# lhoangan/arap_flow

Measured on AMD Instinct MI355X. Metric: ARAP solve+warp frames/sec at 854x480 mesh, higher is better.
Workload: dtype f32; 1 GPU; configs[1]: single 854x480 DAVIS-shaped frame, single-segment mask, fd=1; schedule 19/8/400; segments_per_frame=1, fd=1, parallelism=frames sharded, no collective, grid_vertices_per_frame=409920

## Files before the change

### arap_flow_amd/csrc/arap_resident.h

```cpp
#pragma once
#include <type_traits>
#include "arap_device.h"

namespace arap {

constexpr int RES_WGS = 512;
constexpr int RES_MAX_GROUPS = RES_WGS;
constexpr int RES_THREADS = 256;
constexpr int RES_SLOTS = 9;
constexpr int RES_TILES_PER_WG = RES_SLOTS;
constexpr int RT_X = 32, RT_Y = 8;
constexpr int RES_ZX = 2 * RT_X + 2 * RT_Y;
constexpr int RES_ZG = 2 * RES_ZX;
constexpr int RES_MAX_L = 32000;
static_assert(RT_X * RT_Y == RES_THREADS && RT_Y == 2 * (RES_THREADS / 64), "one vertex per lane, two rows per wavefront");
constexpr int RES_MAX_HALO = RES_TILES_PER_WG * (2 * RT_X + 2 * RT_Y);
constexpr int RES_HALO_PER_THREAD = (RES_MAX_HALO + RES_THREADS - 1) / RES_THREADS;
constexpr int RES_MAX_TILES = RES_WGS * RES_TILES_PER_WG;
constexpr int LROW = RT_X + 2;
constexpr int LROWS = RT_Y + 2;
constexpr int LPLANE = LROW * LROWS;
constexpr int LTILE = 5 * LPLANE;
constexpr int RES_LDS_BYTES = RES_TILES_PER_WG * LTILE * 4
                              + ((RES_MAX_HALO * 8 + 15) / 16) * 16
                              + RES_TILES_PER_WG * 8 + 8 + 384
                              + RES_TILES_PER_WG * RES_ZX * 16;
static_assert(2 * ((RES_LDS_BYTES + 1279) / 1280 * 1280) <= 160 * 1024, "two workgroups per CU");
#ifndef RES_HALO_REG_SLOTS
#define RES_HALO_REG_SLOTS 8
#endif
#ifndef RES_WREG_SLOTS
#define RES_WREG_SLOTS 7
#endif
#ifndef RES_WREG_8
#define RES_WREG_8 4
#endif
#ifndef RES_WREG_9
#define RES_WREG_9 4
#endif
#ifndef RES_WREG_FIT
#define RES_WREG_FIT 9
#endif
#ifndef RES_WREG_FIT_FLAT
#define RES_WREG_FIT_FLAT 9
#endif
#ifndef RES_WPIN
#define RES_WPIN 1
#endif
#ifndef RES_PREG_SLOTS
#define RES_PREG_SLOTS 7
#endif
#ifndef RES_PREG_SLOTS_FLAT
#define RES_PREG_SLOTS_FLAT 7
#endif
#ifndef RES_CSREG_SLOTS
#define RES_CSREG_SLOTS 7
#endif
#ifndef RES_CSREG_SLOTS_FLAT
#define RES_CSREG_SLOTS_FLAT 7
#endif
#ifndef RES_HPREG_SLOTS
#define RES_HPREG_SLOTS 6
#endif
#ifndef RES_HPREG_SLOTS_FLAT
#define RES_HPREG_SLOTS_FLAT 7
#endif
#ifndef RES_SWEEP1
#define RES_SWEEP1 1
#endif
#ifndef RES_WREG_8_FLAT
#define RES_WREG_8_FLAT 4
#endif
#ifndef RES_WREG_9_FLAT
#define RES_WREG_9_FLAT RES_WREG_9
#endif
#ifndef RES_PUB_MASK
#define RES_PUB_MASK 1
#endif
#ifndef RES_Z16
#define RES_Z16 1
#endif
#ifndef RES_FIRST_LOOK
#define RES_FIRST_LOOK 5
#endif
#ifndef RES_FIRST_LOOK_2
#define RES_FIRST_LOOK_2 14
#endif
#ifndef RES_FIRST_LOOK_X
#define RES_FIRST_LOOK_X 20
#endif
#ifndef RES_OWN_LOCAL
#define RES_OWN_LOCAL 1
#endif
#ifndef RES_POLL_SLEEP
#define RES_POLL_SLEEP 1
#endif
constexpr unsigned RES_SPIN_LIMIT = 1u << 18;
#ifndef RES_GRAN_STRIDE
#define RES_GRAN_STRIDE 2
#endif
constexpr int RES_GS = RES_GRAN_STRIDE;
constexpr int RES_GRAN_UNITS = 2 * RES_WGS;
constexpr int RES_GRAN_L1 = 2 * RES_GRAN_UNITS * RES_GS;
constexpr int RES_GRAN2_STRIDE = 16;
constexpr int RES_GRAN2_GROUP = 2 * 8 * RES_GRAN2_STRIDE;
constexpr int RES_GRAN_X = RES_GRAN_L1 + 4 * RES_GRAN2_GROUP;
constexpr int RES_GRAN_PER_LAUNCH = RES_GRAN_X + RES_GRAN_L1;
#ifndef RES_FLAT_MAX_RUNS
#define RES_FLAT_MAX_RUNS 2
#endif

constexpr int RES_SUMS_ANY = 0, RES_SUMS_FLAT = 1, RES_SUMS_COUNT = 2;

struct ResWg {
    int slot;
    int rank;
    int wgs;
    int gran;
};

struct ResDev {
    const int* tilelist;
    const int* ntiles;
    const int* tilepos;
    const int* bandx0;
    unsigned long long* zx;
    int rtX, rtY;
    unsigned long long* gran;
    unsigned* err;
    const ResWg* wgmap;
    int allow_fast;
    int force_fail;
    int flat_runs;
    int nowait;
    int fuse_update;
    unsigned long long* stamps;
};

typedef __attribute__((address_space(1))) unsigned long long gu64;
typedef __attribute__((address_space(1))) unsigned gu32;

__device__ __forceinline__ int border_entry(int x, int y)
{
    return y == 0 ? x : (y == RT_Y - 1 ? RT_X + x : (x == 0 ? 2 * RT_X + y : (x == RT_X - 1 ? 2 * RT_X + RT_Y + y : -1)));
}
__device__ __forceinline__ void st_tagged(unsigned long long* p, unsigned hi , float v, bool fast)
{
    const unsigned long long g = ((unsigned long long)hi << 32) | __float_as_uint(v);
    if (fast) __hip_atomic_store(p, g, __ATOMIC_RELAXED, __HIP_MEMORY_SCOPE_WORKGROUP);
    else __hip_atomic_store(p, g, __ATOMIC_RELAXED, __HIP_MEMORY_SCOPE_AGENT);
}
typedef unsigned v4u_t __attribute__((__vector_size__(4 * sizeof(unsigned))));
__device__ __forceinline__ void ld_zentry(const unsigned long long* zx_b, __amdgpu_buffer_rsrc_t zrs, unsigned gi,
                                          unsigned long long (&h)[2])
{
    if (RES_Z16) {
        const v4u_t w = __builtin_amdgcn_raw_buffer_load_b128(zrs, (int)(gi * 8u), 0, 16 );
        h[0] = ((unsigned long long)w[1] << 32) | w[0];
        h[1] = ((unsigned long long)w[3] << 32) | w[2];
    } else {
        const unsigned long long* q_ = (const unsigned long long*)((const char*)zx_b + (size_t)(gi * 8u));
#pragma unroll
        for (int c = 0; c < 2; ++c) h[c] = __hip_atomic_load(q_ + c, __ATOMIC_RELAXED, __HIP_MEMORY_SCOPE_AGENT);
    }
}
#define RES_GRANULE_FENCE() asm volatile("" ::: "memory")
typedef float v2f_t __attribute__((ext_vector_type(2)));
__device__ __forceinline__ float2 fma2(float2 a, float2 b, float2 c)
{
    const v2f_t r = __builtin_elementwise_fma((v2f_t){a.x, a.y}, (v2f_t){b.x, b.y}, (v2f_t){c.x, c.y});
    return make_float2(r.x, r.y);
}
template <int BITNO>
__device__ __forceinline__ float keep_if(unsigned f, float v)
{
    int m;
    asm("v_bfe_i32 %0, %1, %2, 1" : "=v"(m) : "v"(f), "n"(BITNO));
    return __uint_as_float(__float_as_uint(v) & (unsigned)m);
}

template <int BITNO>
__device__ __forceinline__ float keep_if_here(unsigned f, float v)
{
    int m;
    asm volatile("v_bfe_i32 %0, %1, %2, 1" : "=v"(m) : "v"(f), "n"(BITNO));
    return __uint_as_float(__float_as_uint(v) & (unsigned)m);
}

__device__ __forceinline__ void fma_into(float& p, float b, float z)
{
    asm("v_fma_f32 %0, %1, %0, %2" : "+v"(p) : "v"(b), "v"(z));
}

__device__ __forceinline__ double block_sum_uniform(double t)
{
    return __hiloint2double(__builtin_amdgcn_readlane(__double2hiint(t), 3), __builtin_amdgcn_readlane(__double2loint(t), 3));
}

__device__ __forceinline__ int res_publishes(bool fast, bool flavour)
{
    int s_ = (((threadIdx.x & 63) >> 1) == 1 && fast == flavour) ? 1 : 0;
    asm volatile("" : "+v"(s_));
    return s_;
}

template <bool ONE = false, bool PUBMASK = false>
__device__ __forceinline__ bool group_sum(double part, unsigned epoch, unsigned long long* gran_group, int rank,
                                          int wgs, float* bcast , unsigned* err, float& out,
                                          bool fast = false, double* out_d = nullptr, bool nowait = false,
                                          unsigned long long* tm = nullptr ,
                                          unsigned long long* tarr = nullptr ,
                                          int pubf = 0, int pubs = 0)
{
    const int wave = threadIdx.x >> 6, lane = threadIdx.x & 63;
    unsigned long long c0 = 0ull, c1;
    if (wave == 0) {
        if (tm) c0 = __builtin_amdgcn_s_memtime();
        if (tarr) *tarr += __builtin_amdgcn_s_memrealtime();
        __builtin_amdgcn_s_setprio(3);
        unsigned long long* buf = gran_group + (size_t)(epoch & 1u) * wgs * RES_GS;
        if (PUBMASK) {
            const unsigned long long bits = (unsigned long long)__double_as_longlong(part);
            const unsigned hw = lane == 2 ? (unsigned)bits : (unsigned)(bits >> 32);
            const unsigned long long gv = ((unsigned long long)epoch << 32) | hw;
            if (pubf) __hip_atomic_store(buf + rank * RES_GS + (lane - 2), gv, __ATOMIC_RELAXED, __HIP_MEMORY_SCOPE_WORKGROUP);
            if (pubs) __hip_atomic_store(buf + rank * RES_GS + (lane - 2), gv, __ATOMIC_RELAXED, __HIP_MEMORY_SCOPE_AGENT);
        } else if ((lane >> 1) == 1) {
            const unsigned long long bits = (unsigned long long)__double_as_longlong(part);
            const unsigned hw = lane == 2 ? (unsigned)bits : (unsigned)(bits >> 32);
            const unsigned long long gv = ((unsigned long long)epoch << 32) | hw;
            if (fast)
                __hip_atomic_store(buf + rank * RES_GS + (lane - 2), gv, __ATOMIC_RELAXED, __HIP_MEMORY_SCOPE_WORKGROUP);
            else
                __hip_atomic_store(buf + rank * RES_GS + (lane - 2), gv, __ATOMIC_RELAXED, __HIP_MEMORY_SCOPE_AGENT);
        }
        part = block_sum_uniform(part);
        double v = 0.0;
        bool ok = false;
        if (tm) { c1 = __builtin_amdgcn_s_memtime(); tm[0] += c1 - c0; c0 = c1; }
        __builtin_amdgcn_s_sleep(RES_FIRST_LOOK);
        const bool own1 = RES_OWN_LOCAL && lane == rank;
        const bool look = ONE && lane < wgs && !own1;
        const double idle = own1 ? part : 0.0;
        const __amdgpu_buffer_rsrc_t grs = __builtin_amdgcn_make_buffer_rsrc((void*)gran_group, 0, ONE ? 2 * wgs * RES_GS * 8 : 0, 0x00020000);
        const int qoff = (int)(((epoch & 1u) * (unsigned)wgs + (unsigned)lane) * (RES_GS * 8u));
        v4u_t w = {(unsigned)__double2loint(idle), epoch, (unsigned)__double2hiint(idle), epoch};
        const unsigned limit = nowait ? 1u : RES_SPIN_LIMIT;
        for (unsigned spins = 0; spins < limit; ++spins) {
            if (tm) tm[3] += 1;
            if (ONE) {
                RES_GRANULE_FENCE();
                if (look) w = __builtin_amdgcn_raw_buffer_load_b128(grs, qoff, 0, 16 );
                const bool late = w[1] != epoch || w[3] != epoch;
                v = __hiloint2double((int)w[2], (int)w[0]);
                ok = __builtin_amdgcn_ballot_w64(late) == 0ull;
                if (ok) break;
                if (RES_POLL_SLEEP) __builtin_amdgcn_s_sleep(1);
                continue;
            }
            v = 0.0;
            bool mine_ok = true;
            for (int m = lane; m < wgs; m += 64) {
                const unsigned long long lo = __hip_atomic_load(buf + RES_GS * m, __ATOMIC_RELAXED, __HIP_MEMORY_SCOPE_AGENT);
                const unsigned long long hi =
                    __hip_atomic_load(buf + RES_GS * m + 1, __ATOMIC_RELAXED, __HIP_MEMORY_SCOPE_AGENT);
                const bool own = RES_OWN_LOCAL && m == rank;
                mine_ok = mine_ok && (own || ((unsigned)(lo >> 32) == epoch && (unsigned)(hi >> 32) == epoch));
                v += own ? part : __longlong_as_double((long long)((hi << 32) | (lo & 0xffffffffull)));
            }
            ok = __builtin_amdgcn_ballot_w64(!mine_ok) == 0ull;
            if (ok) break;
            if (RES_POLL_SLEEP) __builtin_amdgcn_s_sleep(1);
        }
        ok = ok || nowait;
        if (tm) { c1 = __builtin_amdgcn_s_memtime(); tm[1] += c1 - c0; c0 = c1; asm volatile("" : "+v"(v)); }
        v = wave_sum_l63_full(v);
        if (tm) {
            asm volatile("" :: "v"(v));
            c1 = __builtin_amdgcn_s_memtime(); tm[4] += c1 - c0;
        }
        if (lane == 63) {
            *(float2*)(bcast + 2 * (epoch & 1u)) = make_float2((float)v, ok ? 1.0f : 0.0f);
            if (out_d) *out_d = v;
            if (!ok) atomicExch(err, 0xDEAD0000u | (epoch & 0xffffu));
        }
        __builtin_amdgcn_s_setprio(0);
        if (tm) { c1 = __builtin_amdgcn_s_memtime(); tm[2] += c1 - c0; c0 = c1; }
    }
    __syncthreads();
    const float2 bc = *(const float2*)(bcast + 2 * (epoch & 1u));
    out = bc.x;
    if (tm && wave == 0) {
        asm volatile("s_waitcnt lgkmcnt(0)" ::: "memory");
        tm[5] += __builtin_amdgcn_s_memtime() - c0;
    }
    return bc.y != 0.0f;
}

__device__ __forceinline__ bool group_sum_h(double part, unsigned epoch, unsigned long long* gran_group,
                                            unsigned long long* gran2 , int rank, int wgs,
                                            float* bcast, unsigned* err, float& out, bool subfast)
{
    const int wave = threadIdx.x >> 6, lane = threadIdx.x & 63;
    if (wave == 0) {
        __builtin_amdgcn_s_setprio(3);
        const int sub = rank >> 6, srank = rank & 63, nsub = wgs >> 6;
        unsigned long long* buf = gran_group + (size_t)sub * (128 * RES_GS) + (size_t)(epoch & 1u) * (64 * RES_GS);
        part = __hiloint2double(__builtin_amdgcn_readfirstlane(__double2hiint(part)),
                                __builtin_amdgcn_readfirstlane(__double2loint(part)));
        if (lane < 2) {
            const unsigned long long bits = (unsigned long long)__double_as_longlong(part);
            const unsigned hw = lane == 0 ? (unsigned)bits : (unsigned)(bits >> 32);
            const unsigned long long gv = ((unsigned long long)epoch << 32) | hw;
            if (subfast)
                __hip_atomic_store(buf + srank * RES_GS + lane, gv, __ATOMIC_RELAXED, __HIP_MEMORY_SCOPE_WORKGROUP);
            else
                __hip_atomic_store(buf + srank * RES_GS + lane, gv, __ATOMIC_RELAXED, __HIP_MEMORY_SCOPE_AGENT);
        }
        double v = 0.0;
        bool ok = false;
// ... 67 lines not shown
                if (subfast)
                    __hip_atomic_store(bufl + srank * RES_GS + lane, gv, __ATOMIC_RELAXED, __HIP_MEMORY_SCOPE_WORKGROUP);
                else
                    __hip_atomic_store(bufl + srank * RES_GS + lane, gv, __ATOMIC_RELAXED, __HIP_MEMORY_SCOPE_AGENT);
            } else {
                __hip_atomic_store(bufx + rank * RES_GS + (lane & 1), gv, __ATOMIC_RELAXED, __HIP_MEMORY_SCOPE_AGENT);
            }
        }
        double v = 0.0;
        bool ok = false;
        __builtin_amdgcn_s_sleep(RES_FIRST_LOOK_X);
        for (unsigned spins = 0; spins < RES_SPIN_LIMIT; ++spins) {
            v = 0.0;
            bool mine_ok = true;
            for (int r = 0; r < nsub; ++r) {
                if (r * 64 + lane >= wgs) break;
                const unsigned long long* src = r == sub ? bufl + RES_GS * lane : bufx + RES_GS * (r * 64 + lane);
                const unsigned long long lo = __hip_atomic_load(src, __ATOMIC_RELAXED, __HIP_MEMORY_SCOPE_AGENT);
                const unsigned long long hi = __hip_atomic_load(src + 1, __ATOMIC_RELAXED, __HIP_MEMORY_SCOPE_AGENT);
                mine_ok = mine_ok && (unsigned)(lo >> 32) == epoch && (unsigned)(hi >> 32) == epoch;
                v += __longlong_as_double((long long)((hi << 32) | (lo & 0xffffffffull)));
            }
            ok = __all(mine_ok);
            if (ok) break;
            if (RES_POLL_SLEEP) __builtin_amdgcn_s_sleep(1);
        }
        v = wave_sum_l63_full(v);
        if (lane == 63) {
            *(float2*)(bcast + 2 * (epoch & 1u)) = make_float2((float)v, ok ? 1.0f : 0.0f);
            if (!ok) atomicExch(err, 0xDEAD4000u | (epoch & 0x3fffu));
        }
        __builtin_amdgcn_s_setprio(0);
    }
    __syncthreads();
    const float2 bc = *(const float2*)(bcast + 2 * (epoch & 1u));
    out = bc.x;
    return bc.y != 0.0f;
}

__device__ __forceinline__ void halo_append(bool take, unsigned short val, unsigned short* hlist, int* nhalo)
{
    const unsigned long long m = __ballot(take);
    if (m == 0ull) return;
    const int first = __builtin_ctzll(m);
    int base = 0;
    if ((int)(threadIdx.x & 63) == first) base = atomicAdd(nhalo, __popcll(m));
    base = __builtin_amdgcn_readlane(base, first);
    const int before = (int)__builtin_amdgcn_mbcnt_hi((unsigned)(m >> 32), __builtin_amdgcn_mbcnt_lo((unsigned)m, 0u));
    if (take) hlist[base + before] = val;
}

__device__ __forceinline__ double block_sum8(double v, double* wsum ,
                                             unsigned long long* tb = nullptr )
{
    static_assert(RES_THREADS / 64 == 4, "one pair sum and one DPP step add four wavefronts");
    unsigned long long c0 = 0ull, c1;
    if (tb) { c0 = __builtin_amdgcn_s_memtime(); asm volatile("" : "+v"(v)); }
    v = wave_sum_l63_full(v);
    if (tb) { asm volatile("" :: "v"(v)); c1 = __builtin_amdgcn_s_memtime(); tb[0] += c1 - c0; c0 = c1; }
    const int wave = threadIdx.x >> 6, lane = threadIdx.x & 63;
    if (lane == 63) wsum[wave] = v;
    __syncthreads();
    double t = 0.0;
    if (wave == 0) {
        const double a = wsum[lane & 3], b = wsum[(lane & 3) ^ 1];
        if (tb) { asm volatile("s_waitcnt lgkmcnt(0)" ::: "memory"); c1 = __builtin_amdgcn_s_memtime(); tb[1] += c1 - c0; c0 = c1; }
        t = dpp_add_f64_full<0x112, 0xf>(a + b);
        if (tb) { asm volatile("" :: "v"(t)); c1 = __builtin_amdgcn_s_memtime(); tb[2] += c1 - c0; }
    }
    return t;
}

template <bool STAMPS, int NS, int SUMS>
__global__ __launch_bounds__(RES_THREADS, 2) void k_pcg_resident(PlanDev pd, ResDev rd, int L)
{
    static_assert(NS >= 1 && NS <= RES_SLOTS, "slots");
    static_assert(SUMS == RES_SUMS_ANY || SUMS == RES_SUMS_FLAT, "group-sum flavour");
    constexpr bool FLAT = SUMS == RES_SUMS_FLAT;
    constexpr bool SPEND = FLAT && !STAMPS;
    constexpr bool ONE_TRIP = FLAT && RES_SWEEP1 != 0;
    constexpr bool PREG = NS <= (FLAT ? RES_PREG_SLOTS_FLAT : RES_PREG_SLOTS);
    constexpr bool CSREG = NS <= (FLAT ? RES_CSREG_SLOTS_FLAT : RES_CSREG_SLOTS) - (STAMPS ? 1 : 0);
    constexpr int WFIT = SPEND ? RES_WREG_FIT_FLAT : RES_WREG_FIT;
    unsigned long long tA = 0, tS1 = 0, tB = 0, tS2 = 0, tU = 0, t0 = 0, t1 = 0;
    unsigned long long tm[6] = {0, 0, 0, 0, 0, 0}, tbs = 0, tzr = 0;
    unsigned long long tbp[3] = {0, 0, 0}, tarr[2] = {0, 0};
#define RES_STAMP(acc) do { if (STAMPS) { t1 = __builtin_amdgcn_s_memrealtime(); acc += t1 - t0; t0 = t1; } } while (0)
    extern __shared__ __attribute__((aligned(16))) float lds[];
    const ResWg me = rd.wgmap[blockIdx.x];
    if (me.slot < 0) return;
    const int rank = me.rank;
    if (rd.force_fail) {
        if (threadIdx.x == 0) atomicExch(rd.err, 0xDEADFFFFu);
        return;
    }
    if (__hip_atomic_load(rd.err, __ATOMIC_RELAXED, __HIP_MEMORY_SCOPE_AGENT) != 0u) return;
    const int b = me.slot;
    const int wgs = me.wgs;
    const int W = pd.W, H = pd.H;
    const size_t gb = (size_t)b * pd.N;
    const int tid = threadIdx.x, lane = tid & 63, wave = tid >> 6;
    const int lx = lane & (RT_X - 1), ly = (wave << 1) | (lane >> 5);
    unsigned short* hlist = (unsigned short*)(lds + RES_TILES_PER_WG * LTILE);
    int2* tbase = (int2*)((char*)hlist + ((RES_MAX_HALO * 8 + 15) / 16) * 16);
    float* moLUT = (float*)(tbase + RES_TILES_PER_WG + 1);
    float* bcast = moLUT + 12;
    int* nhalo = (int*)(bcast + 4);
    double* wsum = (double*)(bcast + 6);
    unsigned* nbits = (unsigned*)(wsum + 10);
    unsigned* nremote = nbits + 16;
    float4* zst = (float4*)((char*)lds + RES_LDS_BYTES - RES_TILES_PER_WG * RES_ZX * 16);
    unsigned long long* gran_group = rd.gran + me.gran;
    unsigned long long* granx_group = FLAT ? nullptr : rd.gran + RES_GRAN_X + me.gran;

    const int nt = rd.ntiles[b];
    const int tbase_n = nt / wgs, textra = nt - tbase_n * wgs;
    const int tp = tbase_n + (rank < textra ? 1 : 0);
    const int tfirst = rank * tbase_n + (rank < textra ? rank : textra);
    const int* tl = rd.tilelist + (size_t)b * RES_MAX_TILES;
    float wr2, wf2;
    {
        const Slot sl = pd.slots[b];
        wr2 = sl.wr * sl.wr;
        wf2 = sl.wf * sl.wf;
        if (tid < 10) {
            const int deg = tid % 5, fit = tid / 5;
            float dO = 0.f;
            for (int k = 0; k < deg; ++k) dO = dO + (sl.wr * sl.wr + sl.wr * sl.wr);
            if (fit) dO = fmaf(sl.wf, sl.wf, dO);
            moLUT[tid] = ginv(dO);
        }
        if (tid == 0) { *nhalo = 0; *nremote = 0u; }
        if (tid < 16) nbits[tid] = 0u;
    }

    float rx[NS], ry[NS], ra[NS];
    float dx_[NS], dy_[NS], da_[NS];
    float apx[NS], apy[NS], apa[NS];
    float ma_[NS], mo_[NS];
    float2 pxy[PREG ? NS : 1];
    float pal[PREG ? NS : 1];
    v2f_t csr[CSREG ? NS : 1];
    float zx_[PREG ? NS : 1], zy_[PREG ? NS : 1], za_[PREG ? NS : 1];
    unsigned fl[NS];
    int ibase[NS];
    constexpr int NWR = NS <= RES_WREG_SLOTS ? 4 : (NS == 8 ? (SPEND ? RES_WREG_8_FLAT : RES_WREG_8)
                                                            : (SPEND ? RES_WREG_9_FLAT : RES_WREG_9));
    constexpr bool WREG = NWR > 0;
    constexpr bool WPIN = WREG && RES_WPIN != 0;
    float we[WREG ? NS : 1][5];
    const int loff = lx + W * ly;

    const int cell = (ly + 1) * LROW + (lx + 1);
#define TP2(T) ((float2*)(T))
#define TCS(T) ((float2*)(T) + LPLANE)
#define TPA(T) ((T) + 4 * LPLANE)

    int org_[NS];
#pragma unroll
    for (int j = 0; j < NS; ++j) org_[j] = j < tp ? tl[tfirst + j] : -1;
    unsigned long long* const zx_b = rd.zx + (size_t)b * RES_MAX_TILES * RES_ZG;
    for (int c = tid; c < tp * RES_ZG; c += RES_THREADS)
        __hip_atomic_store(zx_b + (size_t)tfirst * RES_ZG + c, 0ull, __ATOMIC_RELAXED, __HIP_MEMORY_SCOPE_AGENT);
    const __amdgpu_buffer_rsrc_t zrs = __builtin_amdgcn_make_buffer_rsrc((void*)zx_b, 0, RES_MAX_TILES * RES_ZG * 8, 0x00020000);
    float2 qC[NS], qR[NS], vR[NS], vC[NS], hR[NS], hC[NS];
    float qRa[NS], qM[NS], vRa[NS], vM[NS], hRa[NS], hM[NS];
    unsigned qF[NS], vF[NS], hF[NS];
    const int vrow = ly == 0 ? 0 : RT_Y + 1, hcol = lx == 0 ? 0 : RT_X + 1;
#pragma unroll
    for (int j = 0; j < NS; ++j) {
        qC[j] = qR[j] = vR[j] = vC[j] = hR[j] = hC[j] = make_float2(0.f, 0.f);
        qRa[j] = qM[j] = vRa[j] = vM[j] = hRa[j] = hM[j] = 0.f;
        qF[j] = vF[j] = hF[j] = 0u;
        const int org = org_[j];
        const int y0 = org / W, x0 = org - y0 * W;
        const int x = x0 + lx, y = y0 + ly;
        if (org >= 0 && x < W && y < H) {
            const size_t i = gb + (size_t)(x + W * y);
            qF[j] = pd.flags[i];
            qC[j] = pd.cs[i];
            qR[j] = pd.rO[i]; qRa[j] = pd.rA[i]; qM[j] = pd.preA[i];
            if ((ly == 0 && y0 > 0) || (ly == RT_Y - 1 && y + 1 < H)) {
                const size_t hi = ly == 0 ? i - W : i + W;
                vF[j] = pd.flags[hi]; vR[j] = pd.rO[hi]; vRa[j] = pd.rA[hi]; vM[j] = pd.preA[hi]; vC[j] = pd.cs[hi];
            }
            if ((lx == 0 && x0 > 0) || (lx == RT_X - 1 && x + 1 < W)) {
                const size_t hi = lx == 0 ? i - 1 : i + 1;
                hF[j] = pd.flags[hi]; hR[j] = pd.rO[hi]; hRa[j] = pd.rA[hi]; hM[j] = pd.preA[hi]; hC[j] = pd.cs[hi];
            }
        }
    }
    for (int c = tid; c < NS * LTILE; c += RES_THREADS) lds[c] = 0.f;
    __syncthreads();
#pragma unroll
    for (int j = 0; j < NS; ++j) {
        dx_[j] = dy_[j] = da_[j] = 0.f;
        apx[j] = apy[j] = apa[j] = 0.f;
        const int org = org_[j];
        int x0 = -1, y0 = -1;
        if (org >= 0) { y0 = org / W; x0 = org - y0 * W; }
        float* T = lds + j * LTILE;
        const bool act = (qF[j] & F_ACT) != 0u;
        rx[j] = act ? qR[j].x : 0.f; ry[j] = act ? qR[j].y : 0.f; ra[j] = act ? qRa[j] : 0.f;
        ma_[j] = act ? qM[j] : 0.f;
        mo_[j] = moLUT[__popc(qF[j] & 15u) + 5 * (int)((qF[j] >> 4) & 1u)];
        const float2 p0 = make_float2(mo_[j] * rx[j], mo_[j] * ry[j]);
        const float pa0 = ma_[j] * ra[j];
        if (act) {
            TP2(T)[cell] = p0;
            TCS(T)[cell] = qC[j];
            TPA(T)[cell] = pa0;
        }
        if (PREG) {
            pxy[j] = act ? p0 : make_float2(0.f, 0.f);
            pal[j] = act ? pa0 : 0.f;
        }
        if (CSREG) csr[j] = act ? (v2f_t){qC[j].x, qC[j].y} : (v2f_t){0.f, 0.f};
        if (vF[j] & F_ACT) {
            const int hc = vrow * LROW + (lx + 1);
            const float mo = moLUT[__popc(vF[j] & 15u) + 5 * (int)((vF[j] >> 4) & 1u)];
            TP2(T)[hc] = make_float2(mo * vR[j].x, mo * vR[j].y); TCS(T)[hc] = vC[j]; TPA(T)[hc] = vM[j] * vRa[j];
        }
        if (hF[j] & F_ACT) {
            const int hc = (ly + 1) * LROW + hcol;
            const float mo = moLUT[__popc(hF[j] & 15u) + 5 * (int)((hF[j] >> 4) & 1u)];
            TP2(T)[hc] = make_float2(mo * hR[j].x, mo * hR[j].y); TCS(T)[hc] = hC[j]; TPA(T)[hc] = hM[j] * hRa[j];
        }
        fl[j] = qF[j];
        ibase[j] = __builtin_amdgcn_readfirstlane(x0 + W * y0);
        if (tid == 0) tbase[j] = make_int2(x0, y0);
    }
    float rho = read_scalar(pd.red + ((size_t)b * pd.nslots + 0) * NSHARD);
    __syncthreads();
#pragma unroll
    for (int j = 0; j < NS; ++j) {
        const unsigned f = fl[j];
        if (WREG) {
            if (NWR > 0) we[j][0] = keep_if<0>(f, wr2);
            if (NWR > 1) we[j][1] = keep_if<1>(f, wr2);
            if (NWR > 2) we[j][2] = keep_if<2>(f, wr2);
            if (NWR > 3) we[j][3] = keep_if<3>(f, wr2);
            if (NS <= WFIT) we[j][4] = keep_if<4>(f, wf2);
        }
        halo_append(ly == 0 && (f & F_E3), (unsigned short)(j * LPLANE + 0 * LROW + lx + 1), hlist, nhalo);
        halo_append(ly == RT_Y - 1 && (f & F_E2), (unsigned short)(j * LPLANE + (RT_Y + 1) * LROW + lx + 1), hlist, nhalo);
        halo_append(lx == 0 && (f & F_E1), (unsigned short)(j * LPLANE + (ly + 1) * LROW + 0), hlist, nhalo);
        halo_append(lx == RT_X - 1 && (f & F_E0), (unsigned short)(j * LPLANE + (ly + 1) * LROW + RT_X + 1), hlist, nhalo);
    }
    __syncthreads();
    const int nh = *nhalo;
    uint2* htab = (uint2*)hlist;
    constexpr bool HREG = NS <= RES_HALO_REG_SLOTS;
    uint2 hreg[RES_HALO_PER_THREAD];
    {
        uint2 e[RES_HALO_PER_THREAD];
#pragma unroll
        for (int u = 0; u < RES_HALO_PER_THREAD; ++u) {
            const int c = tid + u * RES_THREADS;
            e[u] = make_uint2(0u, 0u);
            if (c < nh) {
                const int id = hlist[c];
                const int k = id / LPLANE, rem = id - k * LPLANE;
                const int row = rem / LROW, col = rem - row * LROW;
                const int2 tb = tbase[k];
                const int gx = tb.x + col - 1, gy = tb.y + row - 1;
                e[u].y = (unsigned)(k * (LTILE / 2) + rem) | ((unsigned)(k * LTILE + 4 * LPLANE + rem) << 16);
                const int band = gy / RT_Y;
                const int kx = (gx - rd.bandx0[(size_t)b * rd.rtY + band]) / RT_X;
                const int pos = rd.tilepos[((size_t)b * rd.rtY + band) * rd.rtX + (kx < 0 ? 0 : (kx < rd.rtX ? kx : rd.rtX - 1))];
                const int nfull = textra * (tbase_n + 1);
                const int owner = pos < nfull ? pos / (tbase_n + 1) : textra + (pos - nfull) / (tbase_n > 0 ? tbase_n : 1);
                if (pos >= 0 && owner != rank) atomicOr(&nbits[(owner >> 5) & 15], 1u << (owner & 31));
                const int kxc = kx < 0 ? 0 : (kx < rd.rtX ? kx : rd.rtX - 1);
                const int lxo = gx - (rd.bandx0[(size_t)b * rd.rtY + band] + kxc * RT_X), lyo = gy - band * RT_Y;
                const int zpos = border_entry(lxo, lyo);
                (void)row; (void)col;
                e[u].x = (unsigned)((pos < 0 ? 0 : pos) * RES_ZG + 2 * zpos);
            }
        }
        __syncthreads();
#pragma unroll
        for (int u = 0; u < RES_HALO_PER_THREAD; ++u) {
            if (tid + u * RES_THREADS < RES_MAX_HALO) htab[tid + u * RES_THREADS] = e[u];
            hreg[u] = e[u];
        }
    }
    static_assert(RES_TILES_PER_WG * LTILE < 65536 && LTILE % 2 == 0, "halo table packs 16-bit cell offsets");

    unsigned offP[5], offA[5];
    {
        const int dn[5] = {0, 1, -1, LROW, -LROW};
#pragma unroll
        for (int n = 0; n < 5; ++n) {
            offP[n] = (unsigned)(cell + dn[n]) * 8u;
            offA[n] = (unsigned)(cell + dn[n]) * 4u;
            asm volatile("" : "+v"(offP[n]));
            asm volatile("" : "+v"(offA[n]));
        }
    }
    const int zent = border_entry(lx, ly);
    bool alive = true;
    float alpha_last = 0.f;
    asm volatile("s_waitcnt vmcnt(0)" ::: "memory");
    __syncthreads();
    bool fast = false, zfast = false;
    bool hier = false, subfast = false;
    bool hierx = false;
    unsigned long long* const gran2 =
        FLAT ? nullptr : rd.gran + RES_GRAN_L1 + ((((int)(blockIdx.x & 7u) - (me.rank >> 6)) >> 1) & 3) * RES_GRAN2_GROUP;
    {
        const unsigned xcc = __builtin_amdgcn_s_getreg((3 << 11) | (0 << 6) | 20) & 15u;
        float dummy;
        const double mine = (double)xcc + 65536.0 * (double)(xcc * xcc);
        alive = group_sum<ONE_TRIP>(mine, 1u, gran_group, rank, wgs, bcast, rd.err, dummy, false, wsum + 8);
        const double tot = wsum[8];
        const double s2 = floor(tot / 65536.0), s1 = tot - 65536.0 * s2;
        fast = rd.allow_fast && ((double)wgs * s2 == s1 * s1);
        __syncthreads();
        hier = !FLAT && !fast && wgs > 64;
        hierx = hier && (((wgs + 63) >> 6) <= 2 || ((wgs + 63) >> 6) <= rd.flat_runs);
        if (!fast && rd.allow_fast && alive) {
            if (wave == 0) {
                const unsigned long long* buf = gran_group + (size_t)1 * wgs * RES_GS;
                bool remote = false, elsewhere = false;
                for (int m = lane; m < wgs; m += 64) {
                    const bool nb = ((nbits[(m >> 5) & 15] >> (m & 31)) & 1u) != 0u;
                    const bool same_run = hier && (m >> 6) == (rank >> 6);
                    if (nb || same_run) {
                        const unsigned long long lo = __hip_atomic_load(buf + RES_GS * m, __ATOMIC_RELAXED, __HIP_MEMORY_SCOPE_AGENT);
                        const unsigned long long hi = __hip_atomic_load(buf + RES_GS * m + 1, __ATOMIC_RELAXED, __HIP_MEMORY_SCOPE_AGENT);
                        const double val = __longlong_as_double((long long)((hi << 32) | (lo & 0xffffffffull)));
                        const double q2 = floor(val / 65536.0);
                        const bool other = (unsigned)(lo >> 32) != 1u || (unsigned)(hi >> 32) != 1u ||
                                           (unsigned)(val - 65536.0 * q2) != xcc;
                        remote = remote || (nb && other);
                        elsewhere = elsewhere || (same_run && other);
                    }
                }
                const unsigned any_remote = __any(remote) ? 1u : 0u, any_elsewhere = __any(elsewhere) ? 2u : 0u;
                if (lane == 0) *nremote = any_remote | any_elsewhere;
            }
            __syncthreads();
            zfast = (*nremote & 1u) == 0u;
            subfast = !FLAT && hier && (*nremote & 2u) == 0u;
        } else {
            zfast = fast;
        }
        __syncthreads();
    }
#ifndef RES_PRIO_HI
#define RES_PRIO_HI 2
#endif
#ifndef RES_PRIO_TAIL
#define RES_PRIO_TAIL 2
#endif
#define RES_PRIO(J) { if ((J) + RES_PRIO_TAIL >= NS) __builtin_amdgcn_s_setprio(0); else __builtin_amdgcn_s_setprio(RES_PRIO_HI); }
#define RES_PRIO_END() __builtin_amdgcn_s_setprio(0);
    constexpr bool HPREG = HREG && NS <= (FLAT ? RES_HPREG_SLOTS_FLAT : RES_HPREG_SLOTS) - (STAMPS ? 1 : 0);
    float2 hp2[RES_HALO_PER_THREAD];
    float hpa[RES_HALO_PER_THREAD];
    if (HPREG) {
#pragma unroll
        for (int u = 0; u < RES_HALO_PER_THREAD; ++u) {
            hp2[u] = make_float2(0.f, 0.f); hpa[u] = 0.f;
            if (tid + u * RES_THREADS < nh) {
                hp2[u] = *(const float2*)((const char*)lds + (hreg[u].y & 0xffffu) * 8u);
                hpa[u] = *(const float*)((const char*)lds + (hreg[u].y >> 16) * 4u);
            }
        }
    }
    constexpr bool PUBMASK = FLAT && RES_PUB_MASK != 0 && !(STAMPS && NS == RES_SLOTS);
    const int pubf = PUBMASK ? res_publishes(fast, true) : 0, pubs = PUBMASK ? res_publishes(fast, false) : 0;
    const bool zskip = rd.nowait != 0;
    if (STAMPS) t0 = __builtin_amdgcn_s_memrealtime();
    for (int l = 0; l < L && alive; ++l) {
        static_assert(F_E0 == 1u && F_E1 == 2u && F_E2 == 4u && F_E3 == 8u && F_FIT == 16u && F_ACT == 32u, "bit numbers below");
        if (WPIN) {
#pragma unroll
            for (int j = 0; j < NS; ++j)
#pragma unroll
                for (int e_ = 0; e_ < 5; ++e_)
                    if (e_ < NWR || (e_ == 4 && NS <= WFIT)) asm volatile("" : "+v"(we[WREG ? j : 0][e_]));
        }
        if (CSREG) {
#pragma unroll
            for (int j = 0; j < (CSREG ? NS : 0); ++j) asm volatile("" : "+v"(csr[j]));
        }
        double acc = 0.0;
        float2 Lpv[2], Lcs[2], LqO[2][4], Lcn[2][4];
        float Lpa[2], LqA[2][4];
#define RES_LOAD_A(J)                                                                                  \
        {                                                                                              \
            const int s_ = (J) & 1;                                                                    \
            const char* T_ = (const char*)lds + (J) * (LTILE * 4);                                     \
            if (!PREG) Lpv[s_] = *(const float2*)(T_ + offP[0]);                                       \
            if (!CSREG) Lcs[s_] = *(const float2*)(T_ + offP[0] + LPLANE * 8);                         \
            if (!PREG) Lpa[s_] = *(const float*)(T_ + offA[0] + LPLANE * 16);                          \
            _Pragma("unroll") for (int n_ = 0; n_ < 2; ++n_) {                                         \
                LqO[s_][n_] = *(const float2*)(T_ + offP[n_ + 1]);                                     \
                Lcn[s_][n_] = *(const float2*)(T_ + offP[n_ + 1] + LPLANE * 8);                        \
                LqA[s_][n_] = *(const float*)(T_ + offA[n_ + 1] + LPLANE * 16);                        \
            }                                                                                          \
        }
#define RES_LOAD_B(J)                                                                                  \
        {                                                                                              \
            const int s_ = (J) & 1;                                                                    \
            const char* T_ = (const char*)lds + (J) * (LTILE * 4);                                     \
            _Pragma("unroll") for (int n_ = 2; n_ < 4; ++n_) {                                         \
                LqO[s_][n_] = *(const float2*)(T_ + offP[n_ + 1]);                                     \
                Lcn[s_][n_] = *(const float2*)(T_ + offP[n_ + 1] + LPLANE * 8);                        \
                LqA[s_][n_] = *(const float*)(T_ + offA[n_ + 1] + LPLANE * 16);                        \
            }                                                                                          \
        }
        RES_LOAD_A(0)
        RES_LOAD_B(0)
#pragma unroll
        for (int j = 0; j < NS; ++j) {
            RES_PRIO(j)
            unsigned f = fl[j];
            if (NWR < 4 || !(WREG && NS <= WFIT)) asm volatile("" : "+v"(f));
            const int sj = j & 1;
            if (j + 1 < NS) RES_LOAD_A(j + 1)
            __builtin_amdgcn_sched_barrier(0);
            {
                const float2 pv = PREG ? pxy[PREG ? j : 0] : Lpv[sj];
                const float2 csv = CSREG ? make_float2(csr[CSREG ? j : 0].x, csr[CSREG ? j : 0].y) : Lcs[sj];
                const float pa_ = PREG ? pal[PREG ? j : 0] : Lpa[sj];
                const float ci = csv.x, si = csv.y;
                const float2 pa2 = make_float2(pa_, pa_);
                float2 axy = make_float2(0.f, 0.f);
                float aa = 0.f;
#define RES_EDGE(BITNO, E, NQX, NQY, NHX, NHY, QX, QY)                                                 \
                {                                                                                      \
                    const float2 qO = LqO[sj][E], cn2 = Lcn[sj][E];                                    \
                    const float qA = LqA[sj][E];                                                       \
                    const float cn = cn2.x, sn = cn2.y;                                                \
                    const float w = (BITNO < NWR) ? we[WREG ? j : 0][BITNO] : keep_if<BITNO>(f, wr2);  \
                    const float2 e = pv - qO;                                                          \
                    const float2 t = fma2(make_float2(NQX, NQY), pa2, e);                              \
                    const float2 u = fma2(make_float2(NHX, NHY), make_float2(qA, qA), e + t);          \
                    axy = fma2(make_float2(w, w), u, axy);                                             \
                    aa = fmaf(-w, fmaf(QX, t.x, (QY) * t.y), aa);                                      \
                    (void)cn; (void)sn;                                                                \
                }
                RES_EDGE(0, 0,     -si,  ci,   -sn,  cn,    si, -ci)
                RES_EDGE(1, 1,      si, -ci,    sn, -cn,   -si,  ci)
                __builtin_amdgcn_sched_barrier(0);
                if (j + 1 < NS) RES_LOAD_B(j + 1)
                __builtin_amdgcn_sched_barrier(0);
                RES_EDGE(2, 2,     -ci, -si,   -cn, -sn,    ci,  si)
                RES_EDGE(3, 3,      ci,  si,    cn,  sn,   -ci, -si)
#undef RES_EDGE
                {
                    const float wf = (WREG && NS <= WFIT) ? we[WREG ? j : 0][4] : keep_if<4>(f, wf2);
                    axy = fma2(make_float2(wf, wf), pv, axy);
                }
                const float ax = axy.x, ay = axy.y;
                apx[j] = ax; apy[j] = ay; apa[j] = aa;
                acc += (double)dot3(pv.x, pv.y, pa_, ax, ay, aa);
            }
            __builtin_amdgcn_sched_barrier(0);
        }
#undef RES_LOAD_A
#undef RES_LOAD_B
        float sigma;
        RES_PRIO_END()
        RES_STAMP(tA);
        {
            const unsigned long long cb = STAMPS ? __builtin_amdgcn_s_memtime() : 0ull;
            const double bs = block_sum8(acc, wsum, STAMPS ? tbp : nullptr);
            if (STAMPS) tbs += __builtin_amdgcn_s_memtime() - cb;
            alive = (!FLAT && hierx) ? group_sum_x(block_sum_uniform(bs), 2u * l + 2u, gran_group, granx_group, rank, wgs, bcast, rd.err, sigma, subfast)
                  : (!FLAT && hier)  ? group_sum_h(block_sum_uniform(bs), 2u * l + 2u, gran_group, gran2, rank, wgs, bcast, rd.err, sigma, subfast)
                          : group_sum<ONE_TRIP, PUBMASK>(bs, 2u * l + 2u, gran_group, rank, wgs, bcast, rd.err, sigma, fast, nullptr, rd.nowait != 0,
                                      STAMPS ? tm : nullptr, STAMPS ? tarr : nullptr, pubf, pubs);
        }
        asm volatile("" : "+v"(sigma));
        if (!alive) break;
        RES_STAMP(tS1);
        float alpha = 0.f;
        if (sigma > 0.f) alpha = rho / sigma;
        const unsigned ztag = 2u * l + 3u;
#pragma unroll
        for (int j = 0; j < NS; ++j) {
            RES_PRIO(j)
            const float mo = mo_[j], ma = ma_[j];
            rx[j] = fmaf(-alpha, apx[j], rx[j]);
            ry[j] = fmaf(-alpha, apy[j], ry[j]);
            ra[j] = fmaf(-alpha, apa[j], ra[j]);
            const float zx = mo * rx[j], zy = mo * ry[j], za = ma * ra[j];
            if (PREG) { zx_[j] = zx; zy_[j] = zy; za_[j] = za; }
            if (zent >= 0) {
                zst[j * RES_ZX + zent] = make_float4(zx, zy, za, zy);
            }
            const double t_ = (double)keep_if_here<5>(fl[j], dot3(zx, zy, za, rx[j], ry[j], ra[j]));
            if (j == 0) acc = t_; else acc += t_;
            __builtin_amdgcn_sched_barrier(0);
        }
        float rhoNew;
        RES_PRIO_END()
        RES_STAMP(tB);
        {
            const unsigned long long cb = STAMPS ? __builtin_amdgcn_s_memtime() : 0ull;
            const double bs = block_sum8(acc, wsum, STAMPS ? tbp : nullptr);
            if (STAMPS) tbs += __builtin_amdgcn_s_memtime() - cb;
            if (wave != 0) {
                unsigned long long* const out = zx_b + (size_t)tfirst * RES_ZG;
                const float2* const st2 = (const float2*)zst;
                const unsigned sh = (tid & 1) ? 16u : 0u;
                static_assert(((RES_THREADS - 64) & 1) == 0, "a thread keeps the parity of its granules");
                if (zfast) {
                    for (int g = tid - 64; g < tp * RES_ZG; g += RES_THREADS - 64) {
                        const float2 v = st2[g];
                        st_tagged(out + g, (ztag << 16) | ((__float_as_uint(v.y) >> sh) & 0xffffu), v.x, true);
                    }
                } else {
                    for (int g = tid - 64; g < tp * RES_ZG; g += RES_THREADS - 64) {
                        const float2 v = st2[g];
                        st_tagged(out + g, (ztag << 16) | ((__float_as_uint(v.y) >> sh) & 0xffffu), v.x, false);
                    }
                }
            }
            alive = (!FLAT && hierx) ? group_sum_x(block_sum_uniform(bs), 2u * l + 3u, gran_group, granx_group, rank, wgs, bcast, rd.err, rhoNew, subfast)
                  : (!FLAT && hier)  ? group_sum_h(block_sum_uniform(bs), 2u * l + 3u, gran_group, gran2, rank, wgs, bcast, rd.err, rhoNew, subfast)
                          : group_sum<ONE_TRIP, PUBMASK>(bs, 2u * l + 3u, gran_group, rank, wgs, bcast, rd.err, rhoNew, fast, nullptr, rd.nowait != 0,
                                      STAMPS ? tm : nullptr, STAMPS ? tarr + 1 : nullptr, pubf, pubs);
        }
        unsigned long long hg[RES_HALO_PER_THREAD][2];
        unsigned hpk_[HREG ? 1 : RES_HALO_PER_THREAD];
#define RES_HPK(U) (HREG ? hreg[U].y : hpk_[HREG ? 0 : (U)])
#pragma unroll
        for (int u = 0; u < RES_HALO_PER_THREAD; ++u) {
            hg[u][0] = hg[u][1] = (unsigned long long)ztag << 48;
            if (tid + u * RES_THREADS < nh) ld_zentry(zx_b, zrs, HREG ? hreg[u].x : htab[tid + u * RES_THREADS].x, hg[u]);
        }
        if (!alive) break;
        RES_STAMP(tS2);
        float beta = 0.f;
        if (rho > 0.f) beta = rhoNew / rho;
        rho = rhoNew;
        if (l + 1 == L) { alpha_last = alpha; break; }
        if (PREG) {
#pragma unroll
            for (int j = 0; j < (PREG ? NS : 0); ++j) {
                RES_PRIO(j)
                char* T_ = (char*)lds + j * (LTILE * 4);
                dx_[j] = fmaf(alpha, pxy[j].x, dx_[j]);
                dy_[j] = fmaf(alpha, pxy[j].y, dy_[j]);
                da_[j] = fmaf(alpha, pal[j], da_[j]);
                asm volatile("" : "+v"(dx_[j]), "+v"(dy_[j]), "+v"(da_[j]), "+v"(pxy[j].x), "+v"(pxy[j].y), "+v"(pal[j]));
                fma_into(pxy[j].x, beta, zx_[j]);
                fma_into(pxy[j].y, beta, zy_[j]);
                fma_into(pal[j], beta, za_[j]);
                *(float2*)(T_ + offP[0]) = pxy[j];
                *(float*)(T_ + offA[0] + LPLANE * 16) = pal[j];
            }
        } else {
            float2 Up[NS];
            float Ua[NS];
#pragma unroll
            for (int j = 0; j < NS; ++j) {
                const char* T_ = (const char*)lds + j * (LTILE * 4);
                Up[j] = *(const float2*)(T_ + offP[0]);
                Ua[j] = *(const float*)(T_ + offA[0] + LPLANE * 16);
            }
            __builtin_amdgcn_sched_barrier(0);
#pragma unroll
            for (int j = 0; j < NS; ++j) {
                RES_PRIO(j)
                char* T_ = (char*)lds + j * (LTILE * 4);
                const float mo = mo_[j], ma = ma_[j];
                const float zx = mo * rx[j], zy = mo * ry[j], za = ma * ra[j];
                dx_[j] = fmaf(alpha, Up[j].x, dx_[j]);
                dy_[j] = fmaf(alpha, Up[j].y, dy_[j]);
                da_[j] = fmaf(alpha, Ua[j], da_[j]);
                *(float2*)(T_ + offP[0]) = make_float2(fmaf(beta, Up[j].x, zx), fmaf(beta, Up[j].y, zy));
                *(float*)(T_ + offA[0] + LPLANE * 16) = fmaf(beta, Ua[j], za);
            }
        }
        __builtin_amdgcn_sched_barrier(0);
        if (!HPREG) {
#pragma unroll
            for (int u = 0; u < RES_HALO_PER_THREAD; ++u) {
                hp2[u] = make_float2(0.f, 0.f); hpa[u] = 0.f;
                if (!HREG) hpk_[u] = 0u;
                if (tid + u * RES_THREADS < nh) {
                    if (!HREG) hpk_[u] = htab[tid + u * RES_THREADS].y;
                    hp2[u] = *(const float2*)((const char*)lds + (RES_HPK(u) & 0xffffu) * 8u);
                    hpa[u] = *(const float*)((const char*)lds + (RES_HPK(u) >> 16) * 4u);
                }
            }
        }
#pragma unroll
        for (int j = 0; j < NS; ++j)
            if (HREG && !PREG) asm volatile("" : "+v"(dx_[j]), "+v"(dy_[j]), "+v"(da_[j]));
        __builtin_amdgcn_sched_barrier(0);
        {
            const unsigned zt16 = ztag << 16;
            unsigned bad = 0u;
#pragma unroll
            for (int u = 0; u < RES_HALO_PER_THREAD; ++u)
#pragma unroll
                for (int c = 0; c < 2; ++c) bad |= (unsigned)(hg[u][c] >> 32) ^ zt16;
            bool fresh = (bad >> 16) == 0u;
            if (__builtin_amdgcn_ballot_w64(!fresh) != 0ull) if (!zskip) {
                for (unsigned spins = 0; spins < RES_SPIN_LIMIT; ++spins) {
                    if (STAMPS) tzr += 1;
                    RES_GRANULE_FENCE();
                    fresh = true;
#pragma unroll
                    for (int u = 0; u < RES_HALO_PER_THREAD; ++u) {
                        if (tid + u * RES_THREADS < nh) {
                            ld_zentry(zx_b, zrs, HREG ? hreg[u].x : htab[tid + u * RES_THREADS].x, hg[u]);
#pragma unroll
                            for (int c = 0; c < 2; ++c) fresh = fresh && (unsigned)(hg[u][c] >> 48) == ztag;
                        }
                    }
                    if (__builtin_amdgcn_ballot_w64(!fresh) == 0ull) break;
                    __builtin_amdgcn_s_sleep(1);
                }
                if (!fresh) atomicExch(rd.err, 0xDEAD0000u | (ztag & 0xffffu));
            }
        }
#pragma unroll
        for (int u = 0; u < RES_HALO_PER_THREAD; ++u) {
            const float2 hz2_ = make_float2(__uint_as_float((unsigned)hg[u][0]),
                                            __uint_as_float(((unsigned)(hg[u][0] >> 32) & 0xffffu) | ((unsigned)(hg[u][1] >> 32) << 16)));
            const float hz1_ = __uint_as_float((unsigned)hg[u][1]);
            if (tid + u * RES_THREADS < nh) {
                float2* P = (float2*)((char*)lds + (RES_HPK(u) & 0xffffu) * 8u);
                float* A = (float*)((char*)lds + (RES_HPK(u) >> 16) * 4u);
                if (HPREG) {
                    fma_into(hp2[u].x, beta, hz2_.x);
                    fma_into(hp2[u].y, beta, hz2_.y);
                    fma_into(hpa[u], beta, hz1_);
                    *P = hp2[u];
                    *A = hpa[u];
                } else {
                    *P = make_float2(fmaf(beta, hp2[u].x, hz2_.x), fmaf(beta, hp2[u].y, hz2_.y));
                    *A = fmaf(beta, hpa[u], hz1_);
                }
            }
        }
        RES_PRIO_END()
        __syncthreads();
        RES_STAMP(tU);
    }
    if (STAMPS && tid == 0) {
        unsigned long long* o = rd.stamps + (size_t)blockIdx.x * 16;
        o[8] = tbs; o[9] = tm[0]; o[10] = tm[1]; o[11] = tm[2]; o[12] = tm[3]; o[13] = tzr;
        o[0] = tA; o[1] = tS1; o[2] = tB; o[3] = tS2; o[4] = tU; o[5] = (unsigned long long)tp; { unsigned pc = 0; for (int q = 0; q < 16; ++q) pc += __popc(nbits[q]); o[6] = (unsigned long long)nh | ((unsigned long long)pc << 32) | ((unsigned long long)*nremote << 48); } o[7] = (fast ? 1ull : 0ull) | (zfast ? 2ull : 0ull) | (hier ? 4ull : 0ull) | (subfast ? 8ull : 0ull);
        unsigned long long* q = rd.stamps + (size_t)RES_WGS * 16 + (size_t)blockIdx.x * 16;
        q[0] = tbp[0]; q[1] = tbp[1]; q[2] = tbp[2]; q[3] = tm[4]; q[4] = tm[5]; q[5] = tarr[0]; q[6] = tarr[1];
        q[7] = (unsigned long long)__builtin_amdgcn_s_getreg((31 << 11) | (0 << 6) | 4) |
               ((unsigned long long)(__builtin_amdgcn_s_getreg((3 << 11) | (0 << 6) | 20) & 15u) << 32);
        q[8] = (unsigned long long)tp; q[9] = (unsigned long long)nh; q[10] = (unsigned long long)tp * RES_ZG;
        q[11] = (unsigned long long)rank | ((unsigned long long)wgs << 16) | ((unsigned long long)b << 32); q[12] = (unsigned long long)L;
    }
    if (!alive) return;
    if (L > 0) {
#pragma unroll
        for (int j = 0; j < NS; ++j) {
            const char* T_ = (const char*)lds + j * (LTILE * 4);
            const float2 p2 = PREG ? pxy[PREG ? j : 0] : *(const float2*)(T_ + offP[0]);
            const float pa1 = PREG ? pal[PREG ? j : 0] : *(const float*)(T_ + offA[0] + LPLANE * 16);
            dx_[j] = fmaf(alpha_last, p2.x, dx_[j]);
            dy_[j] = fmaf(alpha_last, p2.y, dy_[j]);
            da_[j] = fmaf(alpha_last, pa1, da_[j]);
        }
    }
    int lo = loff;
    asm volatile("" : "+v"(lo));
    if (rd.fuse_update) {
        const Slot sl = pd.slots[b];
        float2 o_[NS];
        float a_[NS];
#pragma unroll
        for (int j = 0; j < NS; ++j) {
            o_[j] = make_float2(0.f, 0.f); a_[j] = 0.f;
            if (fl[j] & F_ACT) { const int i = ibase[j] + lo; o_[j] = sl.O[i]; a_[j] = sl.A[i]; }
        }
#pragma unroll
        for (int j = 0; j < NS; ++j) {
            if (fl[j] & F_ACT) {
                const int i = ibase[j] + lo;
                float2 o = o_[j];
                o.x = o.x + dx_[j];
                o.y = o.y + dy_[j];
                const float a = a_[j] + da_[j];
                sl.O[i] = o;
                sl.A[i] = a;
                pd.cs[gb + i] = sincos_spec(a);
            }
        }
        return;
    }
#pragma unroll
    for (int j = 0; j < NS; ++j) {
        const unsigned f = fl[j];
        if (f & F_ACT) {
            const int i = ibase[j] + lo;
            pd.deltaO[gb + i] = make_float2(dx_[j], dy_[j]);
            pd.deltaA[gb + i] = da_[j];
        }
    }
}

#undef RES_STAMP
#undef RES_GRANULE_FENCE
#undef RES_HPK
#undef RES_PRIO
#undef RES_PRIO_END
#undef TP2
#undef TCS
#undef TPA

}
```

Measured before the change: 36.02 frames/s.

## Interleave position and cos/sin into float4 LDS cells to halve neighbor loads

Changes the per-tile LDS layout so each cell's position pair and cos/sin pair sit in a single 16-byte float4 instead of two separate float2 planes. Neighbor loads in the CG matvec become one ds_read_b128 per neighbor instead of two b64 reads, and the edge formulas are re-signed to match. The z staging store writes only three floats, and the packed publish reads y from the neighboring slot by parity. Halo offsets are updated for the new stride. This cuts LDS instruction count at the cost of wider loads and possible bank-conflict changes.

```diff
diff --git a/arap_flow_amd/csrc/arap_resident.h b/arap_flow_amd/csrc/arap_resident.h
--- a/arap_flow_amd/csrc/arap_resident.h
+++ b/arap_flow_amd/csrc/arap_resident.h
@@ -21,6 +21,7 @@
 constexpr int LROWS = RT_Y + 2;
 constexpr int LPLANE = LROW * LROWS;
 constexpr int LTILE = 5 * LPLANE;
+static_assert((LTILE * 4) % 16 == 0, "every tile's cells are 16-byte aligned");
 constexpr int RES_LDS_BYTES = RES_TILES_PER_WG * LTILE * 4
                               + ((RES_MAX_HALO * 8 + 15) / 16) * 16
                               + RES_TILES_PER_WG * 8 + 8 + 384
@@ -166,6 +167,7 @@
 }
 #define RES_GRANULE_FENCE() asm volatile("" ::: "memory")
 typedef float v2f_t __attribute__((ext_vector_type(2)));
+typedef float v3f_t __attribute__((ext_vector_type(3)));
 __device__ __forceinline__ float2 fma2(float2 a, float2 b, float2 c)
 {
     const v2f_t r = __builtin_elementwise_fma((v2f_t){a.x, a.y}, (v2f_t){b.x, b.y}, (v2f_t){c.x, c.y});
@@ -539,8 +541,7 @@
     const int loff = lx + W * ly;
 
     const int cell = (ly + 1) * LROW + (lx + 1);
-#define TP2(T) ((float2*)(T))
-#define TCS(T) ((float2*)(T) + LPLANE)
+#define TPC(T) ((float4*)(T))
 #define TPA(T) ((T) + 4 * LPLANE)
 
     int org_[NS];
@@ -594,8 +595,7 @@
         const float2 p0 = make_float2(mo_[j] * rx[j], mo_[j] * ry[j]);
         const float pa0 = ma_[j] * ra[j];
         if (act) {
-            TP2(T)[cell] = p0;
-            TCS(T)[cell] = qC[j];
+            TPC(T)[cell] = make_float4(p0.x, p0.y, qC[j].x, qC[j].y);
             TPA(T)[cell] = pa0;
         }
         if (PREG) {
@@ -606,12 +606,12 @@
         if (vF[j] & F_ACT) {
             const int hc = vrow * LROW + (lx + 1);
             const float mo = moLUT[__popc(vF[j] & 15u) + 5 * (int)((vF[j] >> 4) & 1u)];
-            TP2(T)[hc] = make_float2(mo * vR[j].x, mo * vR[j].y); TCS(T)[hc] = vC[j]; TPA(T)[hc] = vM[j] * vRa[j];
+            TPC(T)[hc] = make_float4(mo * vR[j].x, mo * vR[j].y, vC[j].x, vC[j].y); TPA(T)[hc] = vM[j] * vRa[j];
         }
         if (hF[j] & F_ACT) {
             const int hc = (ly + 1) * LROW + hcol;
             const float mo = moLUT[__popc(hF[j] & 15u) + 5 * (int)((hF[j] >> 4) & 1u)];
-            TP2(T)[hc] = make_float2(mo * hR[j].x, mo * hR[j].y); TCS(T)[hc] = hC[j]; TPA(T)[hc] = hM[j] * hRa[j];
+            TPC(T)[hc] = make_float4(mo * hR[j].x, mo * hR[j].y, hC[j].x, hC[j].y); TPA(T)[hc] = hM[j] * hRa[j];
         }
         fl[j] = qF[j];
         ibase[j] = __builtin_amdgcn_readfirstlane(x0 + W * y0);
@@ -651,7 +651,7 @@
                 const int row = rem / LROW, col = rem - row * LROW;
                 const int2 tb = tbase[k];
                 const int gx = tb.x + col - 1, gy = tb.y + row - 1;
-                e[u].y = (unsigned)(k * (LTILE / 2) + rem) | ((unsigned)(k * LTILE + 4 * LPLANE + rem) << 16);
+                e[u].y = (unsigned)(k * (LTILE / 2) + 2 * rem) | ((unsigned)(k * LTILE + 4 * LPLANE + rem) << 16);
                 const int band = gy / RT_Y;
                 const int kx = (gx - rd.bandx0[(size_t)b * rd.rtY + band]) / RT_X;
                 const int pos = rd.tilepos[((size_t)b * rd.rtY + band) * rd.rtX + (kx < 0 ? 0 : (kx < rd.rtX ? kx : rd.rtX - 1))];
@@ -679,7 +679,7 @@
         const int dn[5] = {0, 1, -1, LROW, -LROW};
 #pragma unroll
         for (int n = 0; n < 5; ++n) {
-            offP[n] = (unsigned)(cell + dn[n]) * 8u;
+            offP[n] = (unsigned)(cell + dn[n]) * 16u;
             offA[n] = (unsigned)(cell + dn[n]) * 4u;
             asm volatile("" : "+v"(offP[n]));
             asm volatile("" : "+v"(offA[n]));
@@ -774,30 +774,25 @@
             for (int j = 0; j < (CSREG ? NS : 0); ++j) asm volatile("" : "+v"(csr[j]));
         }
         double acc = 0.0;
-        float2 Lpv[2], Lcs[2], LqO[2][4], Lcn[2][4];
+        float4 Lown[2], Lq[2][4];
+        float2 Lcs[2];
         float Lpa[2], LqA[2][4];
 #define RES_LOAD_A(J)                                                                                  \
         {                                                                                              \
             const int s_ = (J) & 1;                                                                    \
             const char* T_ = (const char*)lds + (J) * (LTILE * 4);                                     \
-            if (!PREG) Lpv[s_] = *(const float2*)(T_ + offP[0]);                                       \
-            if (!CSREG) Lcs[s_] = *(const float2*)(T_ + offP[0] + LPLANE * 8);                         \
+            if (!PREG) Lown[s_] = *(const float4*)(T_ + offP[0]);                                      \
+            else if (!CSREG) Lcs[s_] = *(const float2*)(T_ + offP[0] + 8);                             \
             if (!PREG) Lpa[s_] = *(const float*)(T_ + offA[0] + LPLANE * 16);                          \
-            _Pragma("unroll") for (int n_ = 0; n_ < 2; ++n_) {                                         \
-                LqO[s_][n_] = *(const float2*)(T_ + offP[n_ + 1]);                                     \
-                Lcn[s_][n_] = *(const float2*)(T_ + offP[n_ + 1] + LPLANE * 8);                        \
-                LqA[s_][n_] = *(const float*)(T_ + offA[n_ + 1] + LPLANE * 16);                        \
-            }                                                                                          \
+            _Pragma("unroll") for (int n_ = 0; n_ < 2; ++n_) Lq[s_][n_] = *(const float4*)(T_ + offP[n_ + 1]); \
+            _Pragma("unroll") for (int n_ = 0; n_ < 2; ++n_) LqA[s_][n_] = *(const float*)(T_ + offA[n_ + 1] + LPLANE * 16); \
         }
 #define RES_LOAD_B(J)                                                                                  \
         {                                                                                              \
             const int s_ = (J) & 1;                                                                    \
             const char* T_ = (const char*)lds + (J) * (LTILE * 4);                                     \
-            _Pragma("unroll") for (int n_ = 2; n_ < 4; ++n_) {                                         \
-                LqO[s_][n_] = *(const float2*)(T_ + offP[n_ + 1]);                                     \
-                Lcn[s_][n_] = *(const float2*)(T_ + offP[n_ + 1] + LPLANE * 8);                        \
-                LqA[s_][n_] = *(const float*)(T_ + offA[n_ + 1] + LPLANE * 16);                        \
-            }                                                                                          \
+            _Pragma("unroll") for (int n_ = 2; n_ < 4; ++n_) Lq[s_][n_] = *(const float4*)(T_ + offP[n_ + 1]); \
+            _Pragma("unroll") for (int n_ = 2; n_ < 4; ++n_) LqA[s_][n_] = *(const float*)(T_ + offA[n_ + 1] + LPLANE * 16); \
         }
         RES_LOAD_A(0)
         RES_LOAD_B(0)
@@ -810,33 +805,38 @@
             if (j + 1 < NS) RES_LOAD_A(j + 1)
             __builtin_amdgcn_sched_barrier(0);
             {
-                const float2 pv = PREG ? pxy[PREG ? j : 0] : Lpv[sj];
-                const float2 csv = CSREG ? make_float2(csr[CSREG ? j : 0].x, csr[CSREG ? j : 0].y) : Lcs[sj];
+                const float2 pv = PREG ? pxy[PREG ? j : 0] : make_float2(Lown[sj].x, Lown[sj].y);
+                v2f_t own2 = (v2f_t){Lown[sj].z, Lown[sj].w};
+                if (!PREG) asm("" : "+v"(own2));
+                const float2 csv = CSREG ? make_float2(csr[CSREG ? j : 0].x, csr[CSREG ? j : 0].y)
+                                 : PREG ? Lcs[sj] : make_float2(own2.x, own2.y);
                 const float pa_ = PREG ? pal[PREG ? j : 0] : Lpa[sj];
                 const float ci = csv.x, si = csv.y;
-                const float2 pa2 = make_float2(pa_, pa_);
                 float2 axy = make_float2(0.f, 0.f);
                 float aa = 0.f;
-#define RES_EDGE(BITNO, E, NQX, NQY, NHX, NHY, QX, QY)                                                 \
+#define RES_EDGE(BITNO, E, NQX, NQY, PX, PY, NHX, NHY, AX, AY, QX, QY)                                               \
                 {                                                                                      \
-                    const float2 qO = LqO[sj][E], cn2 = Lcn[sj][E];                                    \
+                    const float2 qO = make_float2(Lq[sj][E].x, Lq[sj][E].y);                           \
+                     \
+                    v2f_t cn2 = (v2f_t){Lq[sj][E].z, Lq[sj][E].w};                                     \
+                    asm("" : "+v"(cn2));                                                               \
                     const float qA = LqA[sj][E];                                                       \
                     const float cn = cn2.x, sn = cn2.y;                                                \
                     const float w = (BITNO < NWR) ? we[WREG ? j : 0][BITNO] : keep_if<BITNO>(f, wr2);  \
                     const float2 e = pv - qO;                                                          \
-                    const float2 t = fma2(make_float2(NQX, NQY), pa2, e);                              \
-                    const float2 u = fma2(make_float2(NHX, NHY), make_float2(qA, qA), e + t);          \
+                    const float2 t = fma2(make_float2(NQX, NQY), make_float2(PX, PY), e);              \
+                    const float2 u = fma2(make_float2(NHX, NHY), make_float2(AX, AY), e + t);          \
                     axy = fma2(make_float2(w, w), u, axy);                                             \
                     aa = fmaf(-w, fmaf(QX, t.x, (QY) * t.y), aa);                                      \
                     (void)cn; (void)sn;                                                                \
                 }
-                RES_EDGE(0, 0,     -si,  ci,   -sn,  cn,    si, -ci)
-                RES_EDGE(1, 1,      si, -ci,    sn, -cn,   -si,  ci)
+                RES_EDGE(0, 0,      si,  ci,  -pa_,  pa_,    sn,  cn,  -qA,  qA,    si, -ci)
+                RES_EDGE(1, 1,      si,  ci,   pa_, -pa_,    sn,  cn,   qA, -qA,   -si,  ci)
                 __builtin_amdgcn_sched_barrier(0);
                 if (j + 1 < NS) RES_LOAD_B(j + 1)
                 __builtin_amdgcn_sched_barrier(0);
-                RES_EDGE(2, 2,     -ci, -si,   -cn, -sn,    ci,  si)
-                RES_EDGE(3, 3,      ci,  si,    cn,  sn,   -ci, -si)
+                RES_EDGE(2, 2,     -ci, -si,   pa_,  pa_,   -cn, -sn,   qA,  qA,    ci,  si)
+                RES_EDGE(3, 3,      ci,  si,   pa_,  pa_,    cn,  sn,   qA,  qA,   -ci, -si)
 #undef RES_EDGE
                 {
                     const float wf = (WREG && NS <= WFIT) ? we[WREG ? j : 0][4] : keep_if<4>(f, wf2);
@@ -878,7 +878,7 @@
             const float zx = mo * rx[j], zy = mo * ry[j], za = ma * ra[j];
             if (PREG) { zx_[j] = zx; zy_[j] = zy; za_[j] = za; }
             if (zent >= 0) {
-                zst[j * RES_ZX + zent] = make_float4(zx, zy, za, zy);
+                *(v3f_t*)(zst + j * RES_ZX + zent) = (v3f_t){zx, zy, za};
             }
             const double t_ = (double)keep_if_here<5>(fl[j], dot3(zx, zy, za, rx[j], ry[j], ra[j]));
             if (j == 0) acc = t_; else acc += t_;
@@ -893,18 +893,19 @@
             if (STAMPS) tbs += __builtin_amdgcn_s_memtime() - cb;
             if (wave != 0) {
                 unsigned long long* const out = zx_b + (size_t)tfirst * RES_ZG;
-                const float2* const st2 = (const float2*)zst;
+                const float* const stv = (const float*)zst;
+                const float* const sty = (tid & 1) ? stv - 1 : stv + 1;
                 const unsigned sh = (tid & 1) ? 16u : 0u;
                 static_assert(((RES_THREADS - 64) & 1) == 0, "a thread keeps the parity of its granules");
                 if (zfast) {
                     for (int g = tid - 64; g < tp * RES_ZG; g += RES_THREADS - 64) {
-                        const float2 v = st2[g];
-                        st_tagged(out + g, (ztag << 16) | ((__float_as_uint(v.y) >> sh) & 0xffffu), v.x, true);
+                        const float vx = stv[2 * g], vy = sty[2 * g];
+                        st_tagged(out + g, (ztag << 16) | ((__float_as_uint(vy) >> sh) & 0xffffu), vx, true);
                     }
                 } else {
                     for (int g = tid - 64; g < tp * RES_ZG; g += RES_THREADS - 64) {
-                        const float2 v = st2[g];
-                        st_tagged(out + g, (ztag << 16) | ((__float_as_uint(v.y) >> sh) & 0xffffu), v.x, false);
+                        const float vx = stv[2 * g], vy = sty[2 * g];
+                        st_tagged(out + g, (ztag << 16) | ((__float_as_uint(vy) >> sh) & 0xffffu), vx, false);
                     }
                 }
             }
@@ -1098,8 +1099,7 @@
 #undef RES_HPK
 #undef RES_PRIO
 #undef RES_PRIO_END
-#undef TP2
-#undef TCS
+#undef TPC
 #undef TPA
 
 }
```

New measurement: 37.11 frames/s (median of 6 runs). 3.0% higher.
